# carlosmwh1985/BspAtom

Measured on AMD Instinct MI355X. Metric: l-channel eigensolves/sec at N_bsp=4096 fp64, higher is better.
Workload: dtype f64; 1 GPU; Hydrogen Coulomb l=0..127, N_bsp=4096, k=9, KIND_GRID=0 rb=800 (BASELINE configs[3]); `value` = weak scaling: 128 l-channels per GPU, 128 in total; channels_total=128, eigenvector_owner_rank=0, collective_calls=0, launched_by=python

## Files before the change

bspatom_amd/csrc/capi.hip:

```cpp
#include <atomic>
#include <new>
#include "capi_internal.h"

using namespace bsp;

namespace bsp {
static std::atomic<int> g_process_device{-1};
int process_device() { return g_process_device.load(); }
int process_device_check(int device)
{
    const int cur = g_process_device.load();
    if (cur >= 0 && cur != device) {
        fprintf(stderr, "bspatom: this process already works on device %d; use one process per GPU (device %d refused)\n", cur, device);
        return BSP_ERR_UNSUPPORTED;
    }
    return BSP_OK;
}
void process_device_latch(int device) { int expect = -1; g_process_device.compare_exchange_strong(expect, device); }

int device_cus()
{
    static const int cus = [] {
        int dev = 0, v = 0;
        return (hipGetDevice(&dev) == hipSuccess && hipDeviceGetAttribute(&v, hipDeviceAttributeMultiprocessorCount, dev) == hipSuccess && v > 0) ? v : 256;
    }();
    return cus;
}

hipError_t LaunchCtx::sync()
{
    hipError_t first = hipSuccess;
    auto wait = [&](hipStream_t s) {
        const hipError_t e = s ? hipStreamSynchronize(s) : hipSuccess;
        if (first == hipSuccess) first = e;
    };
    for (hipStream_t s : cw_aux) wait(s);
    for (const Sy2sbLane &ln : lanes) { wait(ln.main); wait(ln.side); }
    return first;
}

void LaunchCtx::release()
{
    (void)sync();
    auto drop_stream = [](hipStream_t &s) { if (s) (void)hipStreamDestroy(s); s = nullptr; };
    auto drop_event = [](hipEvent_t &e) { if (e) (void)hipEventDestroy(e); e = nullptr; };
    for (hipStream_t &s : cw_aux) drop_stream(s);
    drop_event(cw_fork);
    for (hipEvent_t &e : cw_join) drop_event(e);
    for (Sy2sbLane &ln : lanes) { drop_stream(ln.main); drop_stream(ln.side); drop_event(ln.evA); drop_event(ln.evB); drop_event(ln.done); }
    drop_event(sy_fork);
    (void)hipFree(bis_tail); (void)hipFree(bis_qcnt); (void)hipFree(sb2st_chk);
    bis_tail = nullptr; bis_tail_cap = 0; bis_qcnt = nullptr; sb2st_chk = nullptr;
}
}

namespace {
struct OptName { const char *name; const char *env; int Options::*field; };
const OptName OPT_TABLE[] = {
    {"sb2st_version", "BSP_SB2ST_VERSION", &Options::sb2st_version},
    {"sb2st_ring", "BSP_SB2ST_RING", &Options::sb2st_ring},
    {"sb2st_margin", "BSP_SB2ST_MARGIN", &Options::sb2st_margin},
    {"sb2st_hyst", "BSP_SB2ST_HYST", &Options::sb2st_hyst},
    {"sb2st_lead", "BSP_SB2ST_LEAD", &Options::sb2st_lead},
    {"sb2st_check", "BSP_SB2ST_CHECK", &Options::sb2st_check},
    {"sb2st_diag", "BSP_SB2ST_DIAG", &Options::sb2st_diag},
    {"sb2st_force_abort", "BSP_SB2ST_FORCE_ABORT", &Options::sb2st_force_abort},
    {"sy2sb_groups", "BSP_SY2SB_GROUPS", &Options::sy2sb_groups},
    {"sy2sb_lookahead", "BSP_SY2SB_LOOKAHEAD", &Options::sy2sb_lookahead},
    {"sy2sb_segs", "BSP_SY2SB_SEGS", &Options::sy2sb_segs},
    {"panel_qr", "BSP_PANEL_QR", &Options::panel_qr},
    {"gemm_diag", "BSP_GEMM_DIAG", &Options::gemm_diag},
    {"bisect", "BSP_BISECT", &Options::bisect},
    {"bisect_ept", "BSP_BISECT_EPT", &Options::bisect_ept},
    {"bisect_tail", "BSP_BISECT_TAIL", &Options::bisect_tail},
    {"bisect_secant", "BSP_BISECT_SECANT", &Options::bisect_secant},
    {"bisect_pair", "BSP_BISECT_PAIR", &Options::bisect_pair},
    {"bisect_queue", "BSP_BISECT_QUEUE", &Options::bisect_queue},
    {"bisect_queue_grid", "BSP_BISECT_QUEUE_GRID", &Options::bisect_queue_grid},
    {"bisect_diag", "BSP_BISECT_DIAG", &Options::bisect_diag},
    {"no_eigvec_prefetch", "BSP_NO_EIGVEC_PREFETCH", &Options::no_eigvec_prefetch},
    {"vec_early", "BSP_VEC_EARLY", &Options::vec_early},
    {"vec_own_cu", "BSP_VEC_OWN_CU", &Options::vec_own_cu},
    {"poison_c", "BSP_POISON_C", &Options::poison_c},
    {"sb2sb_mfma", "BSP_SB2SB_MFMA", &Options::sb2sb_mfma},
    {"ktime", "BSP_KTIME", &Options::ktime},
    {"tsqr_regcap", "BSP_TSQR_REGCAP", &Options::tsqr_regcap},
    {"tsqr_max_m", "BSP_TSQR_MAX_M", &Options::tsqr_max_m},
    {"sb16_rows", "BSP_SB16_ROWS", &Options::sb16_rows},
    {"route", "BSP_ROUTE", &Options::route},
    {"cw_onediv", "BSP_CW_ONEDIV", &Options::cw_onediv},
    {"cw_items4", "BSP_CW_ITEMS4", &Options::cw_items4},
    {"cw_bcast", "BSP_CW_BCAST", &Options::cw_bcast},
    {"cw_nw", "BSP_CW_NW", &Options::cw_nw},
    {"cw_ldspad", "BSP_CW_LDSPAD", &Options::cw_ldspad},
    {"cw_ipw", "BSP_CW_IPW", &Options::cw_ipw},
    {"cw_band8", "BSP_CW_BAND8", &Options::cw_band8},
    {"cw_split", "BSP_CW_SPLIT", &Options::cw_split},
    {"cw_diag", "BSP_CW_DIAG", &Options::cw_diag},
    {"s_overlap", "BSP_S_OVERLAP", &Options::s_overlap},
    {"cw_streams", "BSP_CW_STREAMS", &Options::cw_streams},
    {"cw_chunk_min", "BSP_CW_CHUNK_MIN", &Options::cw_chunk_min},
    {"sb8_wgs", "BSP_SB8_WGS", &Options::sb8_wgs},
    {"sbr_phased", "BSP_SBR_PHASED", &Options::sbr_phased},
    {"sbr_lag", "BSP_SBR_LAG", &Options::sbr_lag},
    {"sbr_xdpp", "BSP_SBR_XDPP", &Options::sbr_xdpp},
    {"fused_probe", "BSP_FUSED_PROBE", &Options::fused_probe},
    {"dipole_stage_mb", "BSP_DIPOLE_STAGE_MB", &Options::dipole_stage_mb},
    {"resolvent_stage_mb", "BSP_RESOLVENT_STAGE_MB", &Options::resolvent_stage_mb},
    {"resolvent_slots", "BSP_RESOLVENT_SLOTS", &Options::resolvent_slots},
    {"wf_stage_mb", "BSP_WF_STAGE_MB", &Options::wf_stage_mb},
    {"tdse_stage_mb", "BSP_TDSE_STAGE_MB", &Options::tdse_stage_mb},
    {"tdse_adapt_group", "BSP_TDSE_ADAPT_GROUP", &Options::tdse_adapt_group},
    {"tdse_spline_group", "BSP_TDSE_SPLINE_GROUP", &Options::tdse_spline_group},
    {"tdse_split_group", "BSP_TDSE_SPLIT_GROUP", &Options::tdse_split_group},
};
}

namespace bsp {
Options &opts()
{
    static Options o = [] {
        Options v;
        for (const OptName &t : OPT_TABLE) {
            const char *e = getenv(t.env);
            if (e) v.*(t.field) = (*e == 0) ? 1 : atoi(e);
        }
        return v;
    }();
    return o;
}

namespace {
struct KRec { int slot; hipEvent_t e0, e1; };
std::vector<KRec> g_krecs;
std::vector<hipEvent_t> g_kpool;
hipEvent_t g_kopen[KS_COUNT];
hipEvent_t kevent()
{
    hipEvent_t e = nullptr;
    if (!g_kpool.empty()) { e = g_kpool.back(); g_kpool.pop_back(); }
    else if (hipEventCreate(&e) != hipSuccess) e = nullptr;
    return e;
}
const char *const KSLOT_NAMES[KS_COUNT] = {"gemm2_kernel<128,128,MODE 1> (rank-128 update, syr2k)", "gemm2_kernel<64,128,MODE 2> (symm Y = A22 W)",
                                          "panel_qr2_kernel / panel_qr_kernel", "sy2sb chain: G, K (split-K gemm_kernel + splitk_reduce), form_T, tsmm64 (W, Z)",
                                          "sb2sb_mfma_kernel (band 64 -> 16)", "sbr_rows_kernel<8> / <16> / sb16st_kernel (one-column chase to tridiagonal)", "bisect3_kernel",
                                          "band_cholesky_kernel + std_form_kernel",
                                          "crawford_item_kernel and its set-up kernels (band route: pencil -> band 15)",
                                          "operator_band_kernel (bands of caller-given g(r), g(r) d/dr)",
                                          "tdse_stage_kernel (one Runge-Kutta stage of bspatom_tdse_propagate)"};
}
void ktime_begin(int slot, hipStream_t st)
{
    hipEvent_t e = kevent();
    g_kopen[slot] = e;
    if (e) (void)hipEventRecord(e, st);
}
void ktime_end(int slot, hipStream_t st)
{
    hipEvent_t e0 = g_kopen[slot], e1 = kevent();
    g_kopen[slot] = nullptr;
    if (!e0 || !e1) return;
    (void)hipEventRecord(e1, st);
    g_krecs.push_back({slot, e0, e1});
}
}

extern "C" int bspatom_kernel_times(double *ms, int32_t *launches, int cap)
{
    if (!ms || !launches || cap < KS_COUNT) return BSP_ERR_ARG;
    BSP_HIP(hipDeviceSynchronize());
    for (int i = 0; i < cap; ++i) { ms[i] = 0.0; launches[i] = 0; }
    for (const auto &r : g_krecs) {
        float t = 0.f;
        if (hipEventElapsedTime(&t, r.e0, r.e1) == hipSuccess) { ms[r.slot] += t; launches[r.slot] += 1; }
        g_kpool.push_back(r.e0); g_kpool.push_back(r.e1);
// ... 499 lines not shown
```

bspatom_amd/csrc/common.h:

```cpp
#pragma once
#include <hip/hip_runtime.h>
#include <cstdint>
#include <cstdio>
#include <cstdlib>

#define BSP_OK 0
#define BSP_ERR_HIP (-1)
#define BSP_ERR_ARG (-2)
#define BSP_ERR_BSPLVB (-3)
#define BSP_ERR_NOGPU (-4)
#define BSP_ERR_UNSUPPORTED (-5)

#define BSP_HIP(x)                                                                          \
    do {                                                                                    \
        hipError_t e_ = (x);                                                                \
        if (e_ != hipSuccess) {                                                             \
            fprintf(stderr, "bspatom: HIP error '%s' at %s:%d\n", hipGetErrorString(e_),    \
                    __FILE__, __LINE__);                                                    \
            return BSP_ERR_HIP;                                                             \
        }                                                                                   \
    } while (0)

typedef double double4_t __attribute__((ext_vector_type(4)));

__host__ __device__ inline size_t ab_stride(int npad) { return (size_t)npad * 128 + 1088; }

namespace bsp {

constexpr int SBR_XDPP_DEFAULT = 2;

struct Options {
    int sb2st_version = 0;
    int sb2st_ring = 0;
    int sb2st_margin = 3, sb2st_hyst = 2;
    int sb2st_lead = 0;
    int sb2st_check = 0;
    int sb2st_diag = 0;
    int sb2st_force_abort = 0;
    int sy2sb_groups = 2, sy2sb_lookahead = 1, sy2sb_segs = 0;
    int panel_qr = 3;
    int tsqr_max_m = 2048;
    int tsqr_regcap = 1;
    int gemm_diag = 0;
    int bisect = 3, bisect_ept = 0;
    int bisect_secant = 1;
    int bisect_tail = 1;
    int bisect_pair = 1;
    int bisect_queue = 1;
    int bisect_queue_grid = 0;
    int bisect_diag = 0;
    int no_eigvec_prefetch = 0;
    int vec_early = 1;
    int vec_own_cu = 1;
    int sb2sb_mfma = 1;
    int sb16_rows = 1;
    int poison_c = 0;
    int route = 0;
    int fused_probe = 0;
    int cw_items4 = 1;
    int cw_nw = 1;
    int cw_streams = 2;
    int cw_chunk_min = 1024;
    int s_overlap = 1;
    int cw_diag = 0;
    int cw_split = 0;
    int cw_band8 = 1;
    int sb8_wgs = 0;
    int sbr_phased = 1;
    int sbr_lag = 0;
    int sbr_xdpp = SBR_XDPP_DEFAULT;
    int cw_ipw = 0;
    int cw_ldspad = 0;
    int cw_onediv = 0;
    int cw_bcast = 1;
    int dipole_stage_mb = 0;
    int wf_stage_mb = 0;
    int tdse_stage_mb = 0;
    int tdse_adapt_group = 0;
    int tdse_spline_group = 0;
    int tdse_split_group = 0;
    int resolvent_stage_mb = 0;
    int resolvent_slots = 0;
    int ktime = 0;
};
Options &opts();

int process_device();
int process_device_check(int device);
void process_device_latch(int device);
int device_cus();

template <class K>
inline hipError_t allow_lds(K kernel, size_t bytes)
{
    return hipFuncSetAttribute(reinterpret_cast<const void *>(kernel), hipFuncAttributeMaxDynamicSharedMemorySize, (int)bytes);
}
template <class K>
inline int persistent_slots(K kernel, int threads, size_t lds_bytes, int items, int *slots)
{
    int per_cu = 0;
    const int cus = device_cus();
    BSP_HIP(hipOccupancyMaxActiveBlocksPerMultiprocessor(&per_cu, kernel, threads, lds_bytes));
    const long r = (long)(per_cu > 0 ? per_cu : 1) * (cus > 0 ? cus : 1);
    *slots = (int)(r < items ? r : items);
    return BSP_OK;
}

struct Sy2sbLane {
    hipStream_t main = nullptr, side = nullptr;
    hipEvent_t evA = nullptr, evB = nullptr, done = nullptr;
};
constexpr int SY2SB_MAXG = 4;
struct LaunchCtx {
    hipStream_t cw_aux[3] = {nullptr, nullptr, nullptr};
    hipEvent_t cw_fork = nullptr, cw_join[3] = {nullptr, nullptr, nullptr};
    Sy2sbLane lanes[SY2SB_MAXG];
    hipEvent_t sy_fork = nullptr;
    double2 *bis_tail = nullptr;
    size_t bis_tail_cap = 0;
    unsigned *bis_qcnt = nullptr;
    int *sb2st_chk = nullptr;

    LaunchCtx() = default;
    LaunchCtx(const LaunchCtx &) = delete;
    LaunchCtx &operator=(const LaunchCtx &) = delete;
    ~LaunchCtx() { release(); }
    hipError_t sync();
    void release();
};

enum KSlot { KS_SYR2K = 0, KS_SYMM, KS_PANEL_QR, KS_CHAIN, KS_SB2SB, KS_SB16ST, KS_BISECT, KS_STDFORM, KS_CRAWFORD, KS_OPBAND, KS_TDSE, KS_COUNT };
void ktime_begin(int slot, hipStream_t st);
void ktime_end(int slot, hipStream_t st);
struct KScope {
    int slot; hipStream_t st; bool on;
    KScope(int slot_, hipStream_t st_) : slot(slot_), st(st_), on(opts().ktime != 0) { if (on) ktime_begin(slot, st); }
    ~KScope() { if (on) ktime_end(slot, st); }
};

struct GemmDesc {
    int M, N, K, batch;
    const double *A; long sAm, sAk, bA;
    const double *B; long sBk, sBn, bB;
    double *C; long sCm, sCn, bC;
    double alpha, beta;
    int lower_only;
    int yoff;
    int ksplit;
    int kchunk;
    long bCs;
    int nsb, toff;
    int sbpre[80];
    int sbxy[80];
};
int gemm_f64(const GemmDesc &g, hipStream_t st);
int gemm_splitk_f64(const GemmDesc &g, int splits, double *part, hipStream_t st);
int tsmm64_f64(int m, int batch, const double *A, long lda, long bsA, const double *B, long bsB, double *C, long ldc, long bsC,
// ... 248 lines not shown
```

bspatom_amd/csrc/crawford.hip:

```cpp
#include "common.h"
#include "wave_ops.h"
#include <cstdio>

namespace bsp {
namespace {

constexpr int CB = 8;
constexpr int CBB = CB * CB;
constexpr int CWD = CB * (CB + 1) / 2;
constexpr int CWU = CBB - CWD;
__host__ __device__ constexpr int cw_pk(int i, int j) { return i * (i + 1) / 2 + j; }
__host__ __device__ constexpr int cw_up(int i, int j) { return cw_pk(j - 1, i); }
static_assert(cw_pk(CB - 1, CB - 1) == CWD - 1 && cw_up(CB - 2, CB - 1) == CWU - 1, "the last places of the two triangles");


template <int I, bool ONEDIV>
__device__ __forceinline__ void rq_step(double &x0, double &x1, double (&q)[4], const int g, const int c)
{
    constexpr int LEN = CB + I, GI = I & 3;
    double &xr = (I < 4) ? x0 : x1;
    const double xi = bpermute(xr, GI * 16 + c);
    const double sig = cw_rowsum(c < LEN ? xi * xi : 0.0);
    const double alpha = read_lane(xi, LEN);
    const double a2s = fma(alpha, alpha, sig);
// ... 232 lines not shown
#define CW_L5(M) CW_L4(M), M(4)
#define CW_L6(M) CW_L5(M), M(5)
#define CW_L7(M) CW_L6(M), M(6)
#define CW_L8(M) CW_L7(M), M(7)
#define CW_DOT_CASE(n)                                                                                                               \
    if constexpr (CNT == n)                                                                                                          \
        asm(CW_PAD CW_FD##n : [a0] "+v"(ws[0]), [a1] "+v"(ws[1]), [a2] "+v"(ws[2]), [a3] "+v"(ws[3])                           \
            : CW_L##n(CW_UI), CW_L##n(CW_XI), [I] "i"(I));
#define CW_AXPY_CASE(n)                                                                                                              \
    if constexpr (CNT == n) asm(CW_PAD CW_FA##n : CW_L##n(CW_XO) : CW_L##n(CW_UI), [tw] "v"(tw), [I] "i"(I));
#define CW_AXPYL_CASE(n)                                                                                                             \
    if constexpr (CNT == n)                                                                                                          \
        asm(CW_PAD CW_FA##n "v_fmac_f64 %[xl], %[nt], %[w]\n\t" : CW_L##n(CW_XO), [xl] "+v"(x[O + n])                                  \
            : CW_L##n(CW_UI), [tw] "v"(tw), [nt] "v"(nt), [w] "v"(w), [I] "i"(I));

template <int I, int O, int CNT>
__device__ __forceinline__ void cw_bdot(double (&ws)[4], const double (&u)[16], const double (&x)[16])
{
    static_assert(CNT >= 1 && CNT <= 8 && (O & 3) == 0, "a statement of at most eight FMAs");
    CW_DOT_CASE(1) CW_DOT_CASE(2) CW_DOT_CASE(3) CW_DOT_CASE(4) CW_DOT_CASE(5) CW_DOT_CASE(6) CW_DOT_CASE(7) CW_DOT_CASE(8)
}
template <int I, int O, int CNT>
__device__ __forceinline__ void cw_baxpy(double (&x)[16], const double (&u)[16], const double tw)
{
    static_assert(CNT >= 1 && CNT <= 8, "a statement of at most eight FMAs");
    CW_AXPY_CASE(1) CW_AXPY_CASE(2) CW_AXPY_CASE(3) CW_AXPY_CASE(4) CW_AXPY_CASE(5) CW_AXPY_CASE(6) CW_AXPY_CASE(7) CW_AXPY_CASE(8)
}

template <int I, int O, int CNT>
__device__ __forceinline__ void cw_baxpy_last(double (&x)[16], const double (&u)[16], const double tw, const double nt, const double w)
{
    static_assert(CNT >= 1 && CNT <= 7, "a statement of at most eight FMAs");
    CW_AXPYL_CASE(1) CW_AXPYL_CASE(2) CW_AXPYL_CASE(3) CW_AXPYL_CASE(4) CW_AXPYL_CASE(5) CW_AXPYL_CASE(6) CW_AXPYL_CASE(7)
}

template <int I, bool ONEDIV>
__device__ __forceinline__ void rq4_step_dpp(double (&x)[16], double (&q)[16], const int r)
{
    constexpr int LEN = CB + I;
    double sg[4] = {0.0, 0.0, 0.0, 0.0};
#pragma unroll
    for (int c = 0; c < LEN; ++c) sg[c & 3] = fma(x[c], x[c], sg[c & 3]);
    const double sigl = (sg[0] + sg[1]) + (sg[2] + sg[3]), alphal = x[LEN];
    double sig, alpha;
    asm(CW_PAD
        "v_mov_b64_dpp %[s], %[sl]" CW_DPPC "v_mov_b64_dpp %[a], %[al]" CW_DPPC
        : [s] "=&v"(sig), [a] "=&v"(alpha) : [sl] "v"(sigl), [al] "v"(alphal), [I] "i"(I));
    const double a2s = fma(alpha, alpha, sig);
    const bool ok = (a2s > 1e-280) && (sig != 0.0);
    const double nrm = sqrt(ok ? a2s : 1.0);
    const double bt = (alpha >= 0.0) ? -nrm : nrm;
    const double amb = alpha - bt;
    const double okf = ok ? 1.0 : 0.0, ambs = ok ? amb : 1.0, bts = ok ? bt : 1.0;
    const double sc = ONEDIV ? 1.0 : (1.0 / ambs) * okf;
    const double t = (ONEDIV ? -1.0 / (bts * ambs) : (bts - alpha) / bts) * okf;
    double u[16];
#pragma unroll
    for (int c = 0; c < 16; ++c) u[c] = (c < LEN) ? (ONEDIV ? x[c] : x[c] * sc) : (ONEDIV ? amb : 1.0);
    {
        double ws[4] = {0.0, 0.0, 0.0, 0.0};
        cw_bdot<I, 0, 8>(ws, u, x);
        cw_bdot<I, 8, I + 1>(ws, u, x);
        const double w = (ws[0] + ws[1]) + (ws[2] + ws[3]);
        const double tw = (r <= I) ? -t * w : 0.0;
        cw_baxpy<I, 0, 8>(x, u, tw);
        cw_baxpy<I, 8, I + 1>(x, u, tw);
    }
    {
        double ws[4] = {0.0, 0.0, 0.0, 0.0};
        cw_bdot<I, 0, 8>(ws, u, q);
        cw_bdot<I, 8, I + 1>(ws, u, q);
        const double w = (ws[0] + ws[1]) + (ws[2] + ws[3]);
        const double tw = -t * w;
        cw_baxpy<I, 0, 8>(q, u, tw);
        if constexpr (ONEDIV) {
            cw_baxpy<I, 8, I + 1>(q, u, tw);
        } else {
            if constexpr (I > 0) cw_baxpy_last<I, 8, I>(q, u, tw, -t, w);
            else q[LEN] = fma(-t, w, q[LEN]);
        }
    }
}

template <bool ONEDIV, bool BCAST>
__device__ __forceinline__ void cw_quad(const int N, const int t, const int jlo, int nch, int jel, const int ipw, const int nlh,
                                        const int qstride, const int nlead, const int chan, const int idx0, const int lane,
                                        double *Qsw, double *Bcw, double *Wsw, const double *__restrict__ Qel, double *Dall, double *Eall,
                                        double *Gall, double *Uall, unsigned long long *diag)
{
    unsigned long long ts0 = 0, tsa = 0, tsb = 0, tsc = 0, tsd = 0, tse = 0;
    if (diag) ts0 = __builtin_amdgcn_s_memtime();
    if (chan >= nlh) {
        if (jlo + nch > nlead) nch = nlead > jlo ? nlead - jlo : 0;
        if (jel >= nlead) jel = 0;
    }
    const int items = nch + (jel > 0 ? 1 : 0);
    if (idx0 >= items) return;
    const size_t chn = (size_t)chan * N;
    double *D = Dall + chn * CWD, *E = Eall + chn * CBB, *G = Gall + chn * CBB;

#pragma unroll
    for (int s = 0; s < 4; ++s) {
        const int idx = idx0 + s;
        const int kd = s >= ipw ? 0 : (idx < nch ? 1 : ((idx == nch && jel > 0) ? 2 : 0));
        if (kd != 0) {
            const int jx = kd == 1 ? jlo + idx : jel, p = kd == 2 ? jel - 1 : jx - 2 - (t - 2 * jx);
            const double *srcD = D + (size_t)p * CWD + 2 * lane;
            const double *srcE = E + (size_t)((lane < 32 || p < 1) ? p : p - 1) * CBB + 2 * (lane & 31);
            const unsigned ldsD = (unsigned)(size_t)(__attribute__((address_space(3))) void *)(Wsw + s * 4 * CBB);
            unsigned long long ex;
            asm volatile("s_mov_b32 m0, %3\n\ts_mov_b64 %0, exec\n\ts_bfm_b64 exec, %5, 0\n\tglobal_load_lds_dwordx4 %1, off\n\t"
                         "s_mov_b64 exec, %0\n\ts_mov_b32 m0, %4\n\ts_nop 0\n\tglobal_load_lds_dwordx4 %2, off"
                         : "=&s"(ex) : "v"(srcD), "v"(srcE), "s"(ldsD), "s"(ldsD + 2 * CBB * 8), "i"(CWD) : "memory", "m0");
        }
    }

    double wv[4][4], sdv[4][2];
    auto read_ws = [&]() {
        const int g = lane >> 4, c8 = lane & 7;
        const bool left = (lane & 15) < CB;
        int oa[2], ob[2], om[2];
#pragma unroll
        for (int r = 0; r < 2; ++r) {
            const int R = 4 * r + g;
            const int hi = R > c8 ? R : c8, lo = R > c8 ? c8 : R;
            oa[r] = left ? cw_pk(hi, lo) : 2 * CBB + c8 * CB + R;
            ob[r] = left ? 2 * CBB + R * CB + c8 : CWD + cw_pk(hi, lo);
            om[r] = 3 * CBB + R * CB + c8;
        }
#pragma unroll
        for (int s = 0; s < 4; ++s) {
            const double *W0 = Wsw + s * 4 * CBB;
#pragma unroll
            for (int r = 0; r < 2; ++r) {
                wv[s][r] = W0[oa[r]];
                wv[s][r + 2] = W0[ob[r]];
                sdv[s][r] = W0[om[r]];
            }
        }
    };

    if (idx0 < nch) {
        const int it = lane >> 4, r = lane & 15;
        const int idx = idx0 + it;
        const bool live = idx < nch && it < ipw && r < CB;
        const int j = jlo + (idx < nch ? idx : 0), p = j - 2 - (t - 2 * j);
        double x[16], q[16];
        {
            const double *gp = G + (size_t)p * CBB + (r & 7) * CB, *ep = E + (size_t)(p + 1) * CBB + (r & 7) * CB;
#pragma unroll
            for (int c = 0; c < CB; c += 2) {
                const double2 a = *reinterpret_cast<const double2 *>(gp + c), b = *reinterpret_cast<const double2 *>(ep + c);
                x[c] = live ? a.x : 0.0; x[c + 1] = live ? a.y : 0.0;
                x[CB + c] = live ? b.x : 0.0; x[CB + c + 1] = live ? b.y : 0.0;
            }
        }
#pragma unroll
        for (int c = 0; c < 16; ++c) q[c] = (c == r) ? 1.0 : 0.0;
        if (diag) { asm volatile("s_waitcnt vmcnt(0)" ::: "memory"); tsa = __builtin_amdgcn_s_memtime(); }
        if constexpr (BCAST) {
            rq4_step_dpp<7, ONEDIV>(x, q, r);
            rq4_step_dpp<6, ONEDIV>(x, q, r);
            rq4_step_dpp<5, ONEDIV>(x, q, r);
            rq4_step_dpp<4, ONEDIV>(x, q, r);
            rq4_step_dpp<3, ONEDIV>(x, q, r);
            rq4_step_dpp<2, ONEDIV>(x, q, r);
            rq4_step_dpp<1, ONEDIV>(x, q, r);
            rq4_step_dpp<0, ONEDIV>(x, q, r);
        } else {
            double *bc = Bcw + it * 16;
            rq4_step<7, ONEDIV>(x, q, bc, r);
            rq4_step<6, ONEDIV>(x, q, bc, r);
            rq4_step<5, ONEDIV>(x, q, bc, r);
            rq4_step<4, ONEDIV>(x, q, bc, r);
            rq4_step<3, ONEDIV>(x, q, bc, r);
            rq4_step<2, ONEDIV>(x, q, bc, r);
            rq4_step<1, ONEDIV>(x, q, bc, r);
            rq4_step<0, ONEDIV>(x, q, bc, r);
        }
        if (diag) { asm volatile("s_waitcnt lgkmcnt(0)" ::: "memory"); tsb = __builtin_amdgcn_s_memtime(); }
        if (live) {
            double *ep = E + (size_t)(p + 1) * CBB + r * CB;
#pragma unroll
            for (int c = 0; c < CB; c += 2) *reinterpret_cast<double2 *>(ep + c) = make_double2(x[CB + c], x[CB + c + 1]);
        }
        if constexpr (BCAST) {
            asm volatile("s_waitcnt vmcnt(4)" ::: "memory");
            read_ws();
            asm volatile("" ::: "memory");
        }
        double *qs = Qsw + it * (16 * QLD) + r * QLD;
#pragma unroll
        for (int c = 0; c < 16; c += 2) *reinterpret_cast<double2 *>(qs + c) = make_double2(q[c], q[c + 1]);
    } else if constexpr (BCAST) {
        asm volatile("s_waitcnt vmcnt(0)" ::: "memory");
        read_ws();
    }
    if constexpr (BCAST) asm volatile("s_waitcnt lgkmcnt(0)" ::: "memory");
    else if (idx0 < nch) asm volatile("s_waitcnt vmcnt(4) lgkmcnt(0)" ::: "memory");
    else asm volatile("s_waitcnt vmcnt(0) lgkmcnt(0)" ::: "memory");
    if (diag) tsc = __builtin_amdgcn_s_memtime();
    int idx0b = idx0;
    size_t chnb = chn;
    asm volatile("" : "+s"(idx0b), "+s"(chnb));
    D = Dall + chnb * CWD; E = Eall + chnb * CBB; G = Gall + chnb * CBB;
    double *U0 = Uall + (size_t)chan * CWU;

    const int g = lane >> 4, c = lane & 15, c8 = c & 7;
    const bool left = c < CB;
    int kind[4], jj[4], pp[4];
    int dk[2];
    bool low[2];
#pragma unroll
    for (int r = 0; r < 2; ++r) {
        low[r] = 4 * r + g >= c8;
        dk[r] = (left ? 0 : CWD) + cw_pk(4 * r + g, c8);
    }
    double qe[4], xt[2] = {0.0, 0.0};
    if constexpr (!BCAST) read_ws();
#pragma unroll
    for (int s = 0; s < 4; ++s) {
        const int idx = idx0b + s;
        kind[s] = s >= ipw ? 0 : (idx < nch ? 1 : ((idx == nch && jel > 0) ? 2 : 0));
        jj[s] = kind[s] == 1 ? jlo + idx : (kind[s] == 2 ? jel : jlo + idx0b);
        pp[s] = kind[s] == 2 ? jel - 1 : jj[s] - 2 - (t - 2 * jj[s]);
        if (kind[s] == 0) { jj[s] = jj[0]; pp[s] = pp[0]; }
#pragma unroll
        for (int r = 0; r < 2; ++r) sdv[s][r] = (pp[s] >= 1 && left) ? sdv[s][r] : 0.0;
    }
    int se = -1;
#pragma unroll
    for (int s = 0; s < 4; ++s) if (kind[s] == 2) se = s;
    const bool has_x = se >= 0 && (jel + 1 <= N - 1);
    if (se >= 0) {
        const double *Qj = Qel + ((int)chan >= nlh ? qstride : 0) + (size_t)jel * 256;
#pragma unroll
        for (int r = 0; r < 4; ++r) qe[r] = Qj[(4 * r + g) * 16 + c];
        const double *Ej = E + (size_t)(has_x ? jel : 0) * CBB;
#pragma unroll
        for (int r = 0; r < 2; ++r) {
            const double v = Ej[c8 * CB + 4 * r + g];
            xt[r] = (has_x && left) ? v : 0.0;
        }
    }
    if (diag) { asm volatile("s_waitcnt vmcnt(0)" ::: "memory"); tsd = __builtin_amdgcn_s_memtime(); }
#pragma unroll
    for (int s = 0; s < 4; ++s) {
        if (kind[s] == 0) break;
        const bool elim = kind[s] == 2;
        const int p = pp[s];
        double *D0 = D + (size_t)p * CWD, *E0 = E + (size_t)p * CBB;
        double q[4];
        if (!elim) {
            const double *qs = Qsw + s * (16 * QLD);
#pragma unroll
            for (int r = 0; r < 4; ++r) q[r] = qs[(4 * r + g) * QLD + c];
        } else {
#pragma unroll
            for (int r = 0; r < 4; ++r) q[r] = qe[r];
        }
        double4_t P = {0.0, 0.0, 0.0, 0.0}, Wn = {0.0, 0.0, 0.0, 0.0};
#pragma unroll
        for (int r = 0; r < 4; ++r) P = cw_mfma(wv[s][r], q[r], P);
#pragma unroll
        for (int r = 0; r < 4; ++r) Wn = cw_mfma(q[r], P[r], Wn);
        double4_t O = {0.0, 0.0, 0.0, 0.0};
        O = cw_mfma(q[0], sdv[s][0], O);
        O = cw_mfma(q[1], sdv[s][1], O);
        double wd[4] = {Wn[0], Wn[1], Wn[2], Wn[3]}, od[4] = {O[0], O[1], O[2], O[3]};
        asm("" : "+v"(wd[0]), "+v"(wd[1]), "+v"(wd[2]), "+v"(wd[3]), "+v"(od[0]), "+v"(od[1]), "+v"(od[2]), "+v"(od[3]));
#pragma unroll
        for (int r = 0; r < 2; ++r)
            if (low[r]) D0[dk[r]] = left ? wd[r] : wd[r + 2];
        if (left) {
#pragma unroll
            for (int r = 0; r < 2; ++r) E0[(4 * r + g) * CB + c8] = wd[r + 2];
        }
        if (p == 0) {
#pragma unroll
            for (int r = 0; r < 2; ++r)
                if (left && !low[r]) U0[cw_up(4 * r + g, c8)] = wd[r];
        }
        if (p >= 1 && left) {
            double *Em = E + (size_t)(p - 1) * CBB, *Gm = G + (size_t)(p - 1) * CBB;
#pragma unroll
            for (int r = 0; r < 2; ++r) {
                if (!elim) Em[(4 * r + g) * CB + c8] = od[r];
                Gm[(4 * r + g) * CB + c8] = od[r + 2];
            }
        }
        if (elim && has_x) {
            double4_t T = {0.0, 0.0, 0.0, 0.0};
            T = cw_mfma(q[2], xt[0], T);
            T = cw_mfma(q[3], xt[1], T);
            if (left) {
                double *Ej = E + (size_t)jel * CBB;
#pragma unroll
                for (int r = 0; r < 2; ++r) Ej[c8 * CB + 4 * r + g] = T[r + 2];
            }
        }
    }
    if (diag) {
        tse = __builtin_amdgcn_s_memtime();
        asm volatile("s_waitcnt vmcnt(0)" ::: "memory");
        const unsigned long long tsf = __builtin_amdgcn_s_memtime();
        if (lane == 0) {
            const bool a = tsa != 0;
            atomicAdd(diag + 0, a ? tsa - ts0 : 0ull);
            atomicAdd(diag + 1, a ? tsb - tsa : 0ull);
            atomicAdd(diag + 2, a ? tsc - tsb : tsc - ts0);
            atomicAdd(diag + 3, tsd - tsc);
            atomicAdd(diag + 4, tse - tsd);
            atomicAdd(diag + 5, tsf - tse);
            atomicAdd(diag + 6, tsf - ts0);
            atomicAdd(diag + 7, 1ull);
        }
    }
}

template <bool ONEDIV, int NW, bool BCAST>
__global__ __launch_bounds__(64 * NW, (BCAST ? 16 : 8) / NW) void crawford_item4_kernel(int N, int t, int jlo, int nch, int jel, int ipw, int nlh, int qstride,
                                                            int nlead, const double *__restrict__ Qel, double *Dall, double *Eall, double *Gall,
                                                            double *Uall, unsigned long long *diag)
{
    __builtin_amdgcn_s_setprio(3);
    if (diag && (((blockIdx.x & 7) | (blockIdx.y & 7)) != 0)) diag = nullptr;
    __shared__ __attribute__((aligned(16))) double Qs[NW][4][16 * QLD];
    __shared__ __attribute__((aligned(16))) double Bc[BCAST ? 1 : NW][BCAST ? 1 : 4][BCAST ? 2 : 16];
    __shared__ __attribute__((aligned(16))) double Wsep[BCAST ? 1 : NW][BCAST ? 1 : 4][BCAST ? 2 : 4 * CBB];
    static_assert(16 * QLD >= 4 * CBB, "a slot of Q holds a slot of phase B's operands");
    double *Wsw = BCAST ? &Qs[0][0][0] : &Wsep[0][0][0];
    const int lane = threadIdx.x & 63;
    const int wave = __builtin_amdgcn_readfirstlane(threadIdx.x >> 6);
    cw_quad<ONEDIV, BCAST>(N, t, jlo, nch, jel, ipw, nlh, qstride, nlead, (int)blockIdx.y, (blockIdx.x * NW + wave) * ipw, lane,
                           &Qs[wave][0][0], BCAST ? nullptr : &Bc[wave][0][0], Wsw + wave * (BCAST ? 4 * 16 * QLD : 4 * 4 * CBB), Qel, Dall,
                           Eall, Gall, Uall, diag);
}

__global__ void crawford_flip_kernel(int n, int k, const double *__restrict__ SB, double *__restrict__ SBf)
{
    const int idx = blockIdx.x * blockDim.x + threadIdx.x;
    if (idx >= n * k) return;
    const int d = idx / n, i = idx % n;
    SBf[idx] = (i + d < n) ? SB[(size_t)d * n + (n - 1 - i - d)] : 0.0;
    SBf[(size_t)n * k + idx] = SB[idx];
}

__global__ __launch_bounds__(64) void crawford_setup_kernel(int n, int k, int fstride, int jfirst, const double *__restrict__ UB0,
                                                           double *__restrict__ LiB0, double *__restrict__ Qel0)
{
    __shared__ double Ld[CB][CB + 1], M[CB][CB + 1], Li[CB][CB + 1];
    const int j = jfirst + blockIdx.x, t = threadIdx.x, r = t >> 3, c = t & 7, b = k - 1;
    const double *UBf = UB0 + (size_t)blockIdx.y * k * n;
    double *LiB = LiB0 + (size_t)blockIdx.y * fstride * CBB, *Qel = Qel0 + (size_t)blockIdx.y * fstride * 256;
    const int i = CB * j + r;
    {
        const int ic = CB * j + c, d = r - c;
        double v = 0.0;
        if (i >= n) v = (r == c) ? 1.0 : 0.0;
        else if (d >= 0 && d <= b) v = UBf[(size_t)d * n + ic];
        Ld[r][c] = v;
        const int im = CB * (j - 1) + c, dm = CB + r - c;
        double m = 0.0;
        if (j > 0 && i < n && dm <= b) m = UBf[(size_t)dm * n + im];
        M[r][c] = m;
        Li[r][c] = 0.0;
    }
    __syncthreads();
    if (t < CB) {
        double x[CB];
#pragma unroll
        for (int rr = 0; rr < CB; ++rr) {
            double s = (rr == t) ? 1.0 : 0.0;
#pragma unroll
            for (int kk = 0; kk < CB; ++kk)
                if (kk < rr && kk >= t) s -= Ld[rr][kk] * x[kk];
            x[rr] = (rr >= t) ? s / Ld[rr][rr] : 0.0;
        }
#pragma unroll
        for (int rr = 0; rr < CB; ++rr) Li[rr][t] = x[rr];
    }
    __syncthreads();
    double kv = 0.0;
#pragma unroll
    for (int kk = 0; kk < CB; ++kk) kv += Li[r][kk] * M[kk][c];
    LiB[(size_t)j * CBB + t] = Li[r][c];
    double *Q = Qel + (size_t)j * 256;
    Q[r * 16 + c] = (r == c) ? 1.0 : 0.0;
    Q[c * 16 + CB + r] = -kv;
    Q[(CB + r) * 16 + c] = 0.0;
    Q[(CB + c) * 16 + CB + r] = Li[r][c];
}

__global__ __launch_bounds__(64) void crawford_init_kernel(int n, int k, int N, int nlh, int listride, const double *__restrict__ HBall,
                                                          const double *__restrict__ LiB, double *Dall, double *Eall, double *Uall)
{
    __shared__ double Ds[CB][CB + 1], Es[CB][CB + 1], Ls[CB][CB + 1], Ts[CB][CB + 1];
    const int p = blockIdx.x, t = threadIdx.x, r = t >> 3, c = t & 7, b = k - 1;
    const bool fwd = (int)blockIdx.y >= nlh;
    const double *HB = HBall + (size_t)(fwd ? blockIdx.y - nlh : blockIdx.y) * k * n;
    auto Hf = [&](int i, int i2) -> double {
        const int hi = i > i2 ? i : i2, lo = i > i2 ? i2 : i, d = hi - lo;
        return (hi < n && d <= b) ? HB[(size_t)d * n + (fwd ? lo : n - 1 - hi)] : 0.0;
    };
    double dv = Hf(CB * p + r, CB * p + c), ev = Hf(CB * (p + 1) + r, CB * p + c);
    if (p == 0) {
        Ds[r][c] = dv; Es[r][c] = ev; Ls[r][c] = LiB[(fwd ? listride : 0) + t];
        __syncthreads();
        double s = 0.0, e2 = 0.0;
#pragma unroll
        for (int kk = 0; kk < CB; ++kk) { s += Ls[r][kk] * Ds[kk][c]; e2 += Es[r][kk] * Ls[c][kk]; }
        Ts[r][c] = s;
        __syncthreads();
        s = 0.0;
#pragma unroll
        for (int kk = 0; kk < CB; ++kk) s += Ts[r][kk] * Ls[c][kk];
        dv = s; ev = e2;
    }
    const size_t o = (size_t)blockIdx.y * N + p;
// ... 124 lines not shown
        double vi = 0.0;
#pragma unroll
        for (int c = 0; c <= r; ++c) vi = (i == c) ? v[c] : vi;
#pragma unroll
        for (int c = 0; c < CB; ++c) {
            double y = 0.0;
#pragma unroll
            for (int q = 0; q <= r; ++q) y = fma(v[q], read_lane(a[c], CB + q), y);
            if (isD) a[c] = fma(-tau * vi, y, a[c]);
        }
    }
#pragma unroll
    for (int c = 0; c < CB; ++c) {
        if (isE) rowE[c] = a[c];
        else if (isD && c <= i) recD[cw_pk(i, c)] = a[c];
    }
}

__global__ void crawford_band_kernel(int n, int npad, int N, int hw, int Nh, int Ntot, int nl, const double *__restrict__ Dall,
                                     const double *__restrict__ Eall, double *__restrict__ ABall)
{
    const int idx = blockIdx.x * blockDim.x + threadIdx.x;
    if (idx >= npad * 32) return;
    const int j = idx >> 5, d = idx & 31;
    const size_t ch = blockIdx.y;
    double v = 0.0;
    if (j + d < n && d <= hw) {
        const int ihi = n - 1 - j, ilo = ihi - d;
        const int P = ihi >> 3, Pc = ilo >> 3;
        const int rr = ihi & 7, cc = ilo & 7;
        if (Nh == 0) {
            if (P == Pc) v = Dall[(ch * N + Pc) * CWD + cw_pk(rr, cc)];
            else if (P - Pc == 1) v = Eall[(ch * N + Pc) * CBB + rr * CB + cc];
        } else if (P - Pc <= 1) {
            const size_t b0 = ch * N, b1 = (nl + ch) * N;
            if (P == Pc) v = Pc <= Nh ? Dall[(b0 + Pc) * CWD + cw_pk(rr, cc)]
                                      : Dall[(b1 + Ntot - 1 - P) * CWD + cw_pk(CB - 1 - cc, CB - 1 - rr)];
            else v = Pc <= Nh ? Eall[(b0 + Pc) * CBB + rr * CB + cc] : Eall[(b1 + Ntot - 2 - Pc) * CBB + (CB - 1 - cc) * CB + (CB - 1 - rr)];
        }
    }
    ABall[ch * ab_stride(npad) + (size_t)j * 128 + d] = v;
}

}

size_t crawford_work_bytes(int n, int k, int nl)
{
    const size_t N = (n + CB - 1) / CB;
    return ((size_t)4 * k * n + 2 * n + 2 * N * 256 + 2 * N * CBB + (size_t)3 * nl * 2 * (N + 2) * CBB) * sizeof(double) + 64;
}

void crawford_carve(void *base, int n, int k, int nl, CrawfordWork *w)
{
    const size_t N = (n + CB - 1) / CB;
    double *p = static_cast<double *>(base);
    w->SBf = p; p += (size_t)2 * k * n;
    w->UBf = p; p += (size_t)2 * k * n;
    w->rdiagf = p; p += 2 * n;
    w->Qel = p; p += 2 * N * 256;
    w->LiB = p; p += 2 * N * CBB;
    w->D = p; p += (size_t)nl * 2 * (N + 2) * CBB;
    w->U = w->D + (size_t)nl * 2 * (N + 2) * CWD;
    w->E = p; p += (size_t)nl * 2 * (N + 2) * CBB;
    w->G = p; p += (size_t)nl * 2 * (N + 2) * CBB;
    w->info = reinterpret_cast<int *>(p);
}

bool crawford_supported(int n, int k) { return k >= 2 && k - 1 <= CB && n >= 2 * CB; }

namespace {
struct CwShape { int N, Nl, Nh, Nproc, Ns; bool split; };
CwShape cw_shape(int n)
{
    CwShape c;
    c.N = (n + CB - 1) / CB;
    c.Nl = (opts().cw_split > 0 && n % CB == 0) ? (int)((long)c.N * (opts().cw_split > 50 ? 50 : opts().cw_split) / 100) : 0;
    c.split = c.Nl >= 3 && c.N - c.Nl >= 4;
    if (!c.split) c.Nl = 0;
    c.Nh = c.split ? c.N - c.Nl : 0;
    c.Nproc = c.split ? c.Nh : c.N;
    c.Ns = c.split ? c.Nh + 2 : c.N;
    return c;
}
int cw_chunk_cols(int n) { return n < opts().cw_chunk_min ? n + 128 : ((n + CW_CHUNKS - 1) / CW_CHUNKS + 127) / 128 * 128; }
}

int crawford_prepare(int n, int k, const double *d_SB, const CrawfordWork &w, hipStream_t st, hipEvent_t *evc)
{
    if (!crawford_supported(n, k)) return BSP_ERR_UNSUPPORTED;
    const CwShape c = cw_shape(n);
    const int N = c.N, Nh = c.Nh, Nl = c.Nl;
    int rc;
    BSP_HIP(hipMemsetAsync(w.info, 0, sizeof(int), st));
    hipLaunchKernelGGL(crawford_flip_kernel, dim3((n * k + 255) / 256), dim3(256), 0, st, n, k, d_SB, w.SBf);
    if (c.split) {
        if ((rc = launch_band_cholesky_pair(n, k, CB * Nh, w.SBf, w.UBf, w.rdiagf, w.info, st))) return rc;
        hipLaunchKernelGGL(crawford_setup_kernel, dim3(Nh, 2), dim3(64), 0, st, n, k, N, 0, w.UBf, w.LiB, w.Qel);
        hipLaunchKernelGGL(crawford_cut_setup_kernel, dim3(1), dim3(64), 0, st, n, k, N, Nh, Nl, w.SBf, w.LiB, w.Qel, w.info);
    } else if (evc) {
        const int cc = cw_chunk_cols(n);
        for (int q = 0, j0 = 0; q < CW_CHUNKS; ++q, j0 += cc) {
            if (j0 < n) {
                const int j1 = j0 + cc < n ? j0 + cc : n, b0 = j0 / CB, b1 = j1 < n ? j1 / CB : N;
                if ((rc = launch_band_cholesky_range(n, k, j0, j1, w.SBf, w.UBf, w.rdiagf, w.info, st))) return rc;
                hipLaunchKernelGGL(crawford_setup_kernel, dim3(b1 - b0, 1), dim3(64), 0, st, n, k, N, b0, w.UBf, w.LiB, w.Qel);
            }
            BSP_HIP(hipEventRecord(evc[q], st));
        }
    } else {
        if ((rc = launch_band_cholesky(n, k, w.SBf, w.UBf, w.rdiagf, w.info, st))) return rc;
        hipLaunchKernelGGL(crawford_setup_kernel, dim3(N, 1), dim3(64), 0, st, n, k, N, 0, w.UBf, w.LiB, w.Qel);
    }
    if (evc && c.split)
        for (int q = 0; q < CW_CHUNKS; ++q) BSP_HIP(hipEventRecord(evc[q], st));
    BSP_HIP(hipGetLastError());
    return BSP_OK;
}

int crawford_run(LaunchCtx &cx, int n, int npad, int k, int nl, const double *d_SB, const double *d_HB, const CrawfordWork &w, double *d_AB,
                 hipStream_t st, bool s_prepared, hipEvent_t *evc)
{
    if (!crawford_supported(n, k)) return BSP_ERR_UNSUPPORTED;
    const CwShape c = cw_shape(n);
    const int N = c.N, Nl = c.Nl, Nh = c.Nh, Nproc = c.Nproc, Ns = c.Ns;
    const bool split = c.split;
    const int ny = split ? 2 * nl : nl;
    const int nlead = split ? Nl : 0x7fffffff;
    int rc;
    KScope kt(KS_CRAWFORD, st);
    if (!s_prepared && (rc = crawford_prepare(n, k, d_SB, w, st))) return rc;
    if (!s_prepared) evc = nullptr;
    const int ccb = cw_chunk_cols(n) / CB;
    int waited = 0;
    if (evc) BSP_HIP(hipStreamWaitEvent(st, evc[0], 0));
    hipLaunchKernelGGL(crawford_init_kernel, dim3(Nproc, ny), dim3(64), 0, st, n, k, Ns, nl, N * CBB, d_HB, w.LiB, w.D, w.E, w.U);
    BSP_HIP(hipGetLastError());
    const int qstride = N * 256;
    unsigned long long *dg = nullptr;
    if (opts().cw_diag && opts().cw_items4) {
        BSP_HIP(hipMalloc(reinterpret_cast<void **>(&dg), 8 * sizeof(unsigned long long)));
        BSP_HIP(hipMemsetAsync(dg, 0, 8 * sizeof(unsigned long long), st));
    }
    auto wavefront = [&](int t, int jlo, int nch, int jel, int cy, int c0 = 0, hipStream_t ws = nullptr) {
        if (!ws) ws = st;
        double *gD = w.D + (size_t)c0 * Ns * CWD, *gE = w.E + (size_t)c0 * Ns * CBB, *gG = w.G + (size_t)c0 * Ns * CBB;
        double *gU = w.U + (size_t)c0 * CWU;
        const int items = nch + (jel ? 1 : 0);
        if (opts().cw_items4) {
            const int nw = opts().cw_nw == 4 ? 4 : 1;
            const int ipw = (opts().cw_ipw == 1 || opts().cw_ipw == 2) ? opts().cw_ipw : 4;
            const int waves = (items + ipw - 1) / ipw;
            const dim3 grid((waves + nw - 1) / nw, cy), block(64 * nw);
            const size_t pad = (size_t)opts().cw_ldspad * 1024;
#define CW_LAUNCH4(OD, NWV, BC, G, B, LDS)                                                                                           \
    hipLaunchKernelGGL((crawford_item4_kernel<OD, NWV, BC>), G, B, LDS, ws, Ns, t, jlo, nch, jel, ipw, nl, qstride, nlead, w.Qel, gD, gE, gG, gU, dg)
            if (opts().cw_bcast) {
                if (opts().cw_onediv) CW_LAUNCH4(true, 1, true, dim3(waves, cy), dim3(64), 0);
                else if (nw == 4) CW_LAUNCH4(false, 4, true, grid, block, 0);
                else CW_LAUNCH4(false, 1, true, grid, block, pad);
            } else {
                if (opts().cw_onediv) CW_LAUNCH4(true, 1, false, dim3(waves, cy), dim3(64), 0);
                else if (nw == 4) CW_LAUNCH4(false, 4, false, grid, block, 0);
                else CW_LAUNCH4(false, 1, false, grid, block, pad);
            }
#undef CW_LAUNCH4
        } else {
            const dim3 grid((items + 3) / 4, cy);
            if (opts().cw_onediv) hipLaunchKernelGGL(crawford_item_kernel<true>, grid, dim3(256), 0, ws, Ns, t, jlo, nch, jel, nl, qstride, nlead, w.Qel, gD, gE, gG, gU);
            else hipLaunchKernelGGL(crawford_item_kernel<false>, grid, dim3(256), 0, ws, Ns, t, jlo, nch, jel, nl, qstride, nlead, w.Qel, gD, gE, gG, gU);
        }
    };
    const int tmax = (Nproc >= 3) ? 3 * Nproc - 5 : (Nproc == 2 ? 1 : 0);
    int ngrp = 1;
    if (!split && !dg && opts().cw_streams > 1) {
        ngrp = opts().cw_streams > 4 ? 4 : opts().cw_streams;
        while (ngrp > 1 && nl / ngrp < 16) --ngrp;
    }
    hipStream_t *const aux = cx.cw_aux;
    if (ngrp > 1) {
        if (!cx.cw_fork) BSP_HIP(hipEventCreateWithFlags(&cx.cw_fork, hipEventDisableTiming));
        for (int g = 0; g < ngrp - 1; ++g) {
            if (!aux[g]) BSP_HIP(hipStreamCreateWithFlags(&aux[g], hipStreamNonBlocking));
            if (!cx.cw_join[g]) BSP_HIP(hipEventCreateWithFlags(&cx.cw_join[g], hipEventDisableTiming));
        }
        BSP_HIP(hipEventRecord(cx.cw_fork, st));
        for (int g = 0; g < ngrp - 1; ++g) BSP_HIP(hipStreamWaitEvent(aux[g], cx.cw_fork, 0));
    }
    for (int t = 1; t <= tmax; ++t) {
        const int jel = ((t & 1) && (t + 1) / 2 <= Nproc - 1) ? (t + 1) / 2 : 0;
        const int jlo = (t + 2 + 2) / 3;
        const int jhi = (t / 2 < Nproc - 1) ? t / 2 : Nproc - 1;
        const int nch = (jhi >= jlo && jlo >= 2) ? jhi - jlo + 1 : 0;
        if (nch + (jel ? 1 : 0) == 0) continue;
        if (evc && jel) {
            const int q = jel / ccb < CW_CHUNKS - 1 ? jel / ccb : CW_CHUNKS - 1;
            for (; waited < q; ++waited)
                for (int g = 0; g < ngrp; ++g) BSP_HIP(hipStreamWaitEvent(g == 0 ? st : aux[g - 1], evc[waited + 1], 0));
        }
        for (int g = 0; g < ngrp; ++g) {
            const int c0 = (int)((long)ny * g / ngrp), c1 = (int)((long)ny * (g + 1) / ngrp);
            wavefront(t, jlo, nch, jel, c1 - c0, c0, g == 0 ? st : aux[g - 1]);
        }
    }
    for (int g = 0; g < ngrp - 1; ++g) {
        BSP_HIP(hipEventRecord(cx.cw_join[g], aux[g]));
        BSP_HIP(hipStreamWaitEvent(st, cx.cw_join[g], 0));
    }
    if (evc)
        for (; waited < CW_CHUNKS - 1; ++waited) BSP_HIP(hipStreamWaitEvent(st, evc[waited + 1], 0));
    if (split) {
        hipLaunchKernelGGL(crawford_cut_prep_kernel, dim3(nl), dim3(64), 0, st, Ns, Nh, Nl, nl, N, w.LiB, w.D, w.E);
        wavefront(2 * Nh - 1, 0, 0, Nh, nl);
        for (int sft = 0; sft <= Nh - 2; ++sft) wavefront(2 * Nh + sft, Nh, 1, 0, nl);
    }
    BSP_HIP(hipGetLastError());
    if (dg) {
        unsigned long long h[8];
        BSP_HIP(hipStreamSynchronize(st));
        BSP_HIP(hipMemcpy(h, dg, sizeof(h), hipMemcpyDeviceToHost));
        hipFree(dg);
        const double wv = h[7] ? (double)h[7] : 1.0;
        fprintf(stderr, "crawford_item4_kernel, %llu waves, s_memtime ticks per wave: X arrives %.0f | eight reflectors %.0f | R, Q stored %.0f | "
                        "phase B operands arrive %.0f | congruences issued %.0f | stores leave %.0f | wave %.0f\n", h[7], h[0] / wv, h[1] / wv,
                h[2] / wv, h[3] / wv, h[4] / wv, h[5] / wv, h[6] / wv);
    }
    const bool band8 = opts().cw_band8 != 0;
    if (band8) hipLaunchKernelGGL(crawford_corner_kernel, dim3(ny), dim3(64), 0, st, Ns, w.D, w.E, w.U);
    hipLaunchKernelGGL(crawford_band_kernel, dim3((npad * 32 + 255) / 256, nl), dim3(256), 0, st, n, npad, Ns, band8 ? CB : 2 * CB - 1,
                       Nh, N, nl, w.D, w.E, d_AB);
    BSP_HIP(hipGetLastError());
    return BSP_OK;
}

}
```

Baseline: 2218 eigensolves/s.

## Spread Crawford wavefront phase B across 2 or 4 waves when the front is small

Adds a spread kernel variant in which one workgroup of 2 or 4 waves handles a quad of wavefront items. Wave 0 loads the shared Q and W data, a barrier follows, and then each wave runs the MFMA update for its own subset of items. The variant is picked automatically when the number of quads is below caps scaled by the CU count, so small wavefront steps use more of the GPU. The cost is an extra workgroup barrier, a lower occupancy bound per workgroup, and three more tuning options.

```diff
diff --git a/bspatom_amd/csrc/capi.hip b/bspatom_amd/csrc/capi.hip
--- a/bspatom_amd/csrc/capi.hip
+++ b/bspatom_amd/csrc/capi.hip
@@ -92,6 +92,9 @@
     {"cw_items4", "BSP_CW_ITEMS4", &Options::cw_items4},
     {"cw_bcast", "BSP_CW_BCAST", &Options::cw_bcast},
     {"cw_nw", "BSP_CW_NW", &Options::cw_nw},
+    {"cw_spread", "BSP_CW_SPREAD", &Options::cw_spread},
+    {"cw_spread_cap4", "BSP_CW_SPREAD_CAP4", &Options::cw_spread_cap4},
+    {"cw_spread_cap2", "BSP_CW_SPREAD_CAP2", &Options::cw_spread_cap2},
     {"cw_ldspad", "BSP_CW_LDSPAD", &Options::cw_ldspad},
     {"cw_ipw", "BSP_CW_IPW", &Options::cw_ipw},
     {"cw_band8", "BSP_CW_BAND8", &Options::cw_band8},
diff --git a/bspatom_amd/csrc/common.h b/bspatom_amd/csrc/common.h
--- a/bspatom_amd/csrc/common.h
+++ b/bspatom_amd/csrc/common.h
@@ -73,6 +73,9 @@
     int cw_ldspad = 0;
     int cw_onediv = 0;
     int cw_bcast = 1;
+    int cw_spread = 1;
+    int cw_spread_cap4 = -1;
+    int cw_spread_cap2 = -1;
     int dipole_stage_mb = 0;
     int wf_stage_mb = 0;
     int tdse_stage_mb = 0;
diff --git a/bspatom_amd/csrc/crawford.hip b/bspatom_amd/csrc/crawford.hip
--- a/bspatom_amd/csrc/crawford.hip
+++ b/bspatom_amd/csrc/crawford.hip
@@ -338,12 +338,15 @@
     }
 }
 
-template <bool ONEDIV, bool BCAST>
+template <bool ONEDIV, bool BCAST, int SPREAD = 1>
 __device__ __forceinline__ void cw_quad(const int N, const int t, const int jlo, int nch, int jel, const int ipw, const int nlh,
                                         const int qstride, const int nlead, const int chan, const int idx0, const int lane,
                                         double *Qsw, double *Bcw, double *Wsw, const double *__restrict__ Qel, double *Dall, double *Eall,
-                                        double *Gall, double *Uall, unsigned long long *diag)
-{
+                                        double *Gall, double *Uall, unsigned long long *diag, const int wave = 0)
+{
+    static_assert(SPREAD == 1 || (BCAST && (SPREAD == 2 || SPREAD == 4)), "phase B over 2 or 4 waves: the DPP form only");
+    constexpr int NS = 4 / SPREAD;
+    const int s0 = SPREAD > 1 ? wave * NS : 0;
     unsigned long long ts0 = 0, tsa = 0, tsb = 0, tsc = 0, tsd = 0, tse = 0;
     if (diag) ts0 = __builtin_amdgcn_s_memtime();
     if (chan >= nlh) {
@@ -356,7 +359,8 @@
     double *D = Dall + chn * CWD, *E = Eall + chn * CBB, *G = Gall + chn * CBB;
 
 #pragma unroll
-    for (int s = 0; s < 4; ++s) {
+    for (int k = 0; k < NS; ++k) {
+        const int s = s0 + k;
         const int idx = idx0 + s;
         const int kd = s >= ipw ? 0 : (idx < nch ? 1 : ((idx == nch && jel > 0) ? 2 : 0));
         if (kd != 0) {
@@ -371,7 +375,7 @@
         }
     }
 
-    double wv[4][4], sdv[4][2];
+    double wv[NS][4], sdv[NS][2];
     auto read_ws = [&]() {
         const int g = lane >> 4, c8 = lane & 7;
         const bool left = (lane & 15) < CB;
@@ -385,18 +389,18 @@
             om[r] = 3 * CBB + R * CB + c8;
         }
 #pragma unroll
-        for (int s = 0; s < 4; ++s) {
-            const double *W0 = Wsw + s * 4 * CBB;
+        for (int k = 0; k < NS; ++k) {
+            const double *W0 = Wsw + (s0 + k) * 4 * CBB;
 #pragma unroll
             for (int r = 0; r < 2; ++r) {
-                wv[s][r] = W0[oa[r]];
-                wv[s][r + 2] = W0[ob[r]];
-                sdv[s][r] = W0[om[r]];
+                wv[k][r] = W0[oa[r]];
+                wv[k][r + 2] = W0[ob[r]];
+                sdv[k][r] = W0[om[r]];
             }
         }
     };
 
-    if (idx0 < nch) {
+    if (idx0 < nch && (SPREAD == 1 || wave == 0)) {
         const int it = lane >> 4, r = lane & 15;
         const int idx = idx0 + it;
         const bool live = idx < nch && it < ipw && r < CB;
@@ -455,6 +459,10 @@
     if constexpr (BCAST) asm volatile("s_waitcnt lgkmcnt(0)" ::: "memory");
     else if (idx0 < nch) asm volatile("s_waitcnt vmcnt(4) lgkmcnt(0)" ::: "memory");
     else asm volatile("s_waitcnt vmcnt(0) lgkmcnt(0)" ::: "memory");
+    if constexpr (SPREAD > 1) {
+        __builtin_amdgcn_s_barrier();
+        asm volatile("" ::: "memory");
+    }
     if (diag) tsc = __builtin_amdgcn_s_memtime();
     int idx0b = idx0;
     size_t chnb = chn;
@@ -464,7 +472,7 @@
 
     const int g = lane >> 4, c = lane & 15, c8 = c & 7;
     const bool left = c < CB;
-    int kind[4], jj[4], pp[4];
+    int kind[NS], jj[NS], pp[NS];
     int dk[2];
     bool low[2];
 #pragma unroll
@@ -475,18 +483,18 @@
     double qe[4], xt[2] = {0.0, 0.0};
     if constexpr (!BCAST) read_ws();
 #pragma unroll
-    for (int s = 0; s < 4; ++s) {
-        const int idx = idx0b + s;
-        kind[s] = s >= ipw ? 0 : (idx < nch ? 1 : ((idx == nch && jel > 0) ? 2 : 0));
-        jj[s] = kind[s] == 1 ? jlo + idx : (kind[s] == 2 ? jel : jlo + idx0b);
-        pp[s] = kind[s] == 2 ? jel - 1 : jj[s] - 2 - (t - 2 * jj[s]);
-        if (kind[s] == 0) { jj[s] = jj[0]; pp[s] = pp[0]; }
-#pragma unroll
-        for (int r = 0; r < 2; ++r) sdv[s][r] = (pp[s] >= 1 && left) ? sdv[s][r] : 0.0;
+    for (int k = 0; k < NS; ++k) {
+        const int s = s0 + k, idx = idx0b + s;
+        kind[k] = s >= ipw ? 0 : (idx < nch ? 1 : ((idx == nch && jel > 0) ? 2 : 0));
+        jj[k] = kind[k] == 1 ? jlo + idx : (kind[k] == 2 ? jel : jlo + idx0b);
+        pp[k] = kind[k] == 2 ? jel - 1 : jj[k] - 2 - (t - 2 * jj[k]);
+        if (kind[k] == 0) { jj[k] = jj[0]; pp[k] = pp[0]; }
+#pragma unroll
+        for (int r = 0; r < 2; ++r) sdv[k][r] = (pp[k] >= 1 && left) ? sdv[k][r] : 0.0;
     }
     int se = -1;
 #pragma unroll
-    for (int s = 0; s < 4; ++s) if (kind[s] == 2) se = s;
+    for (int k = 0; k < NS; ++k) if (kind[k] == 2) se = k;
     const bool has_x = se >= 0 && (jel + 1 <= N - 1);
     if (se >= 0) {
         const double *Qj = Qel + ((int)chan >= nlh ? qstride : 0) + (size_t)jel * 256;
@@ -501,14 +509,14 @@
     }
     if (diag) { asm volatile("s_waitcnt vmcnt(0)" ::: "memory"); tsd = __builtin_amdgcn_s_memtime(); }
 #pragma unroll
-    for (int s = 0; s < 4; ++s) {
-        if (kind[s] == 0) break;
-        const bool elim = kind[s] == 2;
-        const int p = pp[s];
+    for (int k = 0; k < NS; ++k) {
+        if (kind[k] == 0) break;
+        const bool elim = kind[k] == 2;
+        const int p = pp[k];
         double *D0 = D + (size_t)p * CWD, *E0 = E + (size_t)p * CBB;
         double q[4];
         if (!elim) {
-            const double *qs = Qsw + s * (16 * QLD);
+            const double *qs = Qsw + (s0 + k) * (16 * QLD);
 #pragma unroll
             for (int r = 0; r < 4; ++r) q[r] = qs[(4 * r + g) * QLD + c];
         } else {
@@ -517,12 +525,12 @@
         }
         double4_t P = {0.0, 0.0, 0.0, 0.0}, Wn = {0.0, 0.0, 0.0, 0.0};
 #pragma unroll
-        for (int r = 0; r < 4; ++r) P = cw_mfma(wv[s][r], q[r], P);
+        for (int r = 0; r < 4; ++r) P = cw_mfma(wv[k][r], q[r], P);
 #pragma unroll
         for (int r = 0; r < 4; ++r) Wn = cw_mfma(q[r], P[r], Wn);
         double4_t O = {0.0, 0.0, 0.0, 0.0};
-        O = cw_mfma(q[0], sdv[s][0], O);
-        O = cw_mfma(q[1], sdv[s][1], O);
+        O = cw_mfma(q[0], sdv[k][0], O);
+        O = cw_mfma(q[1], sdv[k][1], O);
         double wd[4] = {Wn[0], Wn[1], Wn[2], Wn[3]}, od[4] = {O[0], O[1], O[2], O[3]};
         asm("" : "+v"(wd[0]), "+v"(wd[1]), "+v"(wd[2]), "+v"(wd[3]), "+v"(od[0]), "+v"(od[1]), "+v"(od[2]), "+v"(od[3]));
 #pragma unroll
@@ -591,6 +599,21 @@
     cw_quad<ONEDIV, BCAST>(N, t, jlo, nch, jel, ipw, nlh, qstride, nlead, (int)blockIdx.y, (blockIdx.x * NW + wave) * ipw, lane,
                            &Qs[wave][0][0], BCAST ? nullptr : &Bc[wave][0][0], Wsw + wave * (BCAST ? 4 * 16 * QLD : 4 * 4 * CBB), Qel, Dall,
                            Eall, Gall, Uall, diag);
+}
+
+template <bool ONEDIV, int SPREAD>
+__global__ __launch_bounds__(64 * SPREAD, 16 / SPREAD) void crawford_item4_spread_kernel(int N, int t, int jlo, int nch, int jel, int nlh, int qstride,
+                                                            int nlead, const double *__restrict__ Qel, double *Dall, double *Eall, double *Gall,
+                                                            double *Uall, unsigned long long *diag)
+{
+    __builtin_amdgcn_s_setprio(3);
+    const int lane = threadIdx.x & 63;
+    const int wave = __builtin_amdgcn_readfirstlane(threadIdx.x >> 6);
+    if (diag && (wave != 0 || ((blockIdx.x & 7) | (blockIdx.y & 7)) != 0)) diag = nullptr;
+    __shared__ __attribute__((aligned(16))) double Qs[4][16 * QLD];
+    __shared__ __attribute__((aligned(16))) double Wop[4][4 * CBB];
+    cw_quad<ONEDIV, true, SPREAD>(N, t, jlo, nch, jel, 4, nlh, qstride, nlead, (int)blockIdx.y, (int)blockIdx.x * 4, lane, &Qs[0][0], nullptr,
+                                  &Wop[0][0], Qel, Dall, Eall, Gall, Uall, diag, wave);
 }
 
 __global__ void crawford_flip_kernel(int n, int k, const double *__restrict__ SB, double *__restrict__ SBf)
@@ -881,6 +904,7 @@
     c.Ns = c.split ? c.Nh + 2 : c.N;
     return c;
 }
+constexpr long CW_SPREAD_CAP4 = 1024, CW_SPREAD_CAP2 = 2048;
 int cw_chunk_cols(int n) { return n < opts().cw_chunk_min ? n + 128 : ((n + CW_CHUNKS - 1) / CW_CHUNKS + 127) / 128 * 128; }
 }
 
@@ -951,6 +975,24 @@
             const int waves = (items + ipw - 1) / ipw;
             const dim3 grid((waves + nw - 1) / nw, cy), block(64 * nw);
             const size_t pad = (size_t)opts().cw_ldspad * 1024;
+            int spread = 1;
+            if (opts().cw_spread > 0 && opts().cw_bcast && nw == 1 && ipw == 4 && !split) {
+                if (opts().cw_spread == 2 || opts().cw_spread == 4) spread = opts().cw_spread;
+                else {
+                    const long quads = (long)waves * ny, cus = device_cus();
+                    const long cap4 = opts().cw_spread_cap4 >= 0 ? opts().cw_spread_cap4 : CW_SPREAD_CAP4 * cus / 256;
+                    const long cap2 = opts().cw_spread_cap2 >= 0 ? opts().cw_spread_cap2 : CW_SPREAD_CAP2 * cus / 256;
+                    spread = quads <= cap4 ? 4 : (quads <= cap2 ? 2 : 1);
+                }
+            }
+            if (spread > 1) {
+#define CW_LAUNCHS(OD, S)                                                                                                            \
+    hipLaunchKernelGGL((crawford_item4_spread_kernel<OD, S>), dim3(waves, cy), dim3(64 * S), 0, ws, Ns, t, jlo, nch, jel, nl, qstride, nlead, w.Qel, gD, gE, gG, gU, dg)
+                if (opts().cw_onediv) { if (spread == 4) CW_LAUNCHS(true, 4); else CW_LAUNCHS(true, 2); }
+                else { if (spread == 4) CW_LAUNCHS(false, 4); else CW_LAUNCHS(false, 2); }
+#undef CW_LAUNCHS
+                return;
+            }
 #define CW_LAUNCH4(OD, NWV, BC, G, B, LDS)                                                                                           \
     hipLaunchKernelGGL((crawford_item4_kernel<OD, NWV, BC>), G, B, LDS, ws, Ns, t, jlo, nch, jel, ipw, nl, qstride, nlead, w.Qel, gD, gE, gG, gU, dg)
             if (opts().cw_bcast) {
```

Result: faster. 2244 eigensolves/s, median of 6 (+1.2%).
